# Gaussian-Splatting-Toolkit/Gaussian-Splatting-Toolkit

Measured on AMD Instinct MI355X. Metric: raster fwd+bwd Mpix/s @1080p (1M Gaussians, SH3), higher is better.
Workload: dtype f32; 1 GPU; 1000000 random Gaussians (SURVEY 8d, seed 42, scales log-U[0.0025,0.025]), SH degree 3, 1920x1080, block 16, fwd+bwd through the rasterizer autograd API; gaussians=1000000, visible=869029, list_entries=4459433, scene=uniform, cpu_bind=cpus 8-15 of NUMA node 0 (GPU 0000:0d:00.0), parallelism=single

## Files before the change

### gaussian-splatting-toolkit_amd/csrc/sort_bucket.hip

```cpp
#include "gsr_common.h"
#include "raster_common.h"
#include "tile_rows.h"

#include <algorithm>

namespace gsr_bsort {

constexpr int kChunk = 4096;
constexpr int kCap = 2048;
constexpr int kWaveCap = 1024;
constexpr int kElemBits = 12;
constexpr int kHistThreads = 1024;
constexpr int kScatterWaves = 4, kScatterThreads = 64 * kScatterWaves, kScatterItems = kChunk / kScatterThreads;
constexpr int kSortThreads = 256;

__device__ __forceinline__ unsigned depth_key(const float *__restrict__ depths, const int *__restrict__ radii,
                                              const int i) {
  const int r = radii[i];
  const unsigned bits = __float_as_uint(depths[i]);
  return r > 0 ? (bits & 0x7fffffffu) : 0u;
}

__device__ __forceinline__ void wave_minmax(unsigned &lo, unsigned &hi) {
#pragma unroll
  for (int o = 32; o > 0; o >>= 1) {
    lo = min(lo, (unsigned)__shfl_xor((int)lo, o));
    hi = max(hi, (unsigned)__shfl_xor((int)hi, o));
  }
}

__device__ __forceinline__ unsigned long long match_digit(const unsigned d, const int bits, const bool live) {
  const unsigned long long all = __ballot(live);
  unsigned lo = (unsigned)all, hi = (unsigned)(all >> 32);
#pragma unroll
  for (int bit = 0; bit < 8; ++bit) {
    if (bit < bits) {
      const unsigned one = (d >> bit) & 1u;
      const unsigned long long set = __ballot(one != 0u);
      const unsigned flip = one - 1u;
      lo &= (unsigned)set ^ flip, hi &= (unsigned)(set >> 32) ^ flip;
    }
  }
  return ((unsigned long long)hi << 32) | lo;
}

struct OctaveMap {
  unsigned base_w;
  unsigned mlo, span;
  float c;
};
constexpr unsigned kMinWidth = 16;
constexpr int kSample = 4096;

__device__ __forceinline__ unsigned bucket_of(const unsigned key, const OctaveMap *__restrict__ map) {
  if (!key) return 0u;
  const OctaveMap t = map[key >> 23];
  const unsigned mant = key & 0x7fffffu, W = t.base_w >> 16, base = t.base_w & 0xffffu;
  const unsigned d = min(mant > t.mlo ? mant - t.mlo : 0u, t.span - 1u);
  return base + min(W - 1u, (unsigned)((float)d * t.c));
}

template <int kT>
__device__ __forceinline__ void load_samples(const int n, const float *__restrict__ depths,
                                             const int *__restrict__ radii, unsigned (&sample)[kSample / kT]) {
  const int spacing = n / (kSample / 16);
#pragma unroll
  for (int q = 0; q < kSample / kT; ++q) {
    const int j = q * kT + (int)threadIdx.x;
    sample[q] = depth_key(depths, radii, (j >> 4) * spacing + (j & 15));
  }
}

template <int kT>
__device__ __forceinline__ void build_bucket_map(const unsigned (&sample)[kSample / kT], const int log2_buckets,
                                                 OctaveMap *__restrict__ map, unsigned *__restrict__ oct,
                                                 int *__restrict__ sh ) {
  const int tid = threadIdx.x, lane = tid & 63, w = tid >> 6;
  const unsigned B = 1u << log2_buckets;
  if (tid < 256) oct[tid] = 0u;
  if (tid == 0) sh[16] = -1, sh[17] = 0;
  __syncthreads();
#pragma unroll
  for (int q = 0; q < kSample / kT; ++q) {
    const unsigned long long peers = match_digit(sample[q] >> 23, 8, sample[q] != 0u);
    if (sample[q] && (peers & ((1ull << lane) - 1ull)) == 0) atomicAdd(&oct[sample[q] >> 23], (unsigned)__popcll(peers));
  }
  __syncthreads();
  {
    unsigned kmin = 0xffffffffu, kmax = 0u;
#pragma unroll
    for (int q = 0; q < kSample / kT; ++q)
      if (sample[q]) kmin = min(kmin, sample[q]), kmax = max(kmax, sample[q]);
    wave_minmax(kmin, kmax);
    if (lane == 0) atomicMin(reinterpret_cast<unsigned *>(&sh[16]), kmin), atomicMax(reinterpret_cast<unsigned *>(&sh[17]), kmax);
  }
  unsigned pop = 0;
  int first = 256, last = -1;
  if (tid < 256) {
    pop = oct[tid];
    if (pop) first = last = tid;
    unsigned sum = pop;
#pragma unroll
    for (int o = 32; o > 0; o >>= 1) {
      first = min(first, __shfl_xor(first, o));
      last = max(last, __shfl_xor(last, o));
      sum += __shfl_xor(sum, o);
    }
    if (lane == 0) sh[w] = first, sh[4 + w] = last, sh[8 + w] = (int)sum;
  }
  __syncthreads();
  first = min(min(sh[0], sh[1]), min(sh[2], sh[3]));
  last = max(max(sh[4], sh[5]), max(sh[6], sh[7]));
  const unsigned visible = (unsigned)max(sh[8] + sh[9] + sh[10] + sh[11], 1);
  int lo = max(first - 1, 0), hi = min(last + 1, 255);
  if (last < 0) lo = 1, hi = 0;
  const unsigned budget = B - 3u - kMinWidth * (unsigned)(hi - lo + 1);
  const bool inside = tid >= lo && tid <= hi;
  const unsigned width =
      (tid < 256 && inside) ? kMinWidth + (unsigned)(((unsigned long long)pop * budget) / visible) : 0u;
  unsigned incl = width;
#pragma unroll
  for (int o = 1; o < 64; o <<= 1) {
    const unsigned t = __shfl_up(incl, o);
    if (lane >= o) incl += t;
  }
  __syncthreads();
  if (tid < 256 && lane == 63) sh[w] = (int)incl;
  __syncthreads();
  if (tid < 256) {
    unsigned base = 2u + incl - width;
    for (int q = 0; q < w; ++q) base += (unsigned)sh[q];
    OctaveMap t{(1u << 16) | (tid > hi ? B - 1u : 1u), 0u, 1u, 0.f};
    if (inside) {
      const unsigned kmin = (unsigned)sh[16], kmax = (unsigned)sh[17];
      unsigned m0 = 0u, m1 = 0x7fffffu;
      if (tid == first) m0 = kmin & 0x7fffffu;
      if (tid == last) m1 = kmax & 0x7fffffu;
      const unsigned pad = (m1 - m0 + 1u) >> 5;
      if (tid == first) m0 = m0 > pad ? m0 - pad : 0u;
      if (tid == last) m1 = min(m1 + pad, 0x7fffffu);
      t.base_w = (width << 16) | base;
      t.mlo = m0, t.span = m1 - m0 + 1u;
      t.c = (float)width / (float)t.span;
    }
    map[tid] = t;
  }
  __syncthreads();
}

struct RecordArgs {
  const float *xys, *conics, *opacities;
  int tiles_x, tiles_y;
  SplatRec *recs;
};

template <bool kRecords>
__global__ __launch_bounds__(kHistThreads) void hist_kernel(const int n, const float *__restrict__ depths,
                                                            const int *__restrict__ radii, const int log2_buckets,
                                                            unsigned *__restrict__ table,
                                                            OctaveMap *__restrict__ map_out, const RecordArgs ra,
                                                            unsigned *__restrict__ zero, const int zero_words) {
  extern __shared__ unsigned h[];
  __shared__ OctaveMap map[256];
  __shared__ unsigned oct[256];
  __shared__ int sh[24];
  constexpr int kI = kChunk / kHistThreads;
  const int tid = threadIdx.x, B = 1 << log2_buckets;
  const int base = blockIdx.x * kChunk;
  for (int z = blockIdx.x * kHistThreads + tid; z < zero_words; z += gridDim.x * kHistThreads) zero[z] = 0u;
  unsigned key[kI];
  SplatIn in[kRecords ? kI : 1];
#pragma unroll
  for (int i = 0; i < kI; ++i) {
    const int idx = base + i * kHistThreads + tid;
    const unsigned k = depth_key(depths, radii, min(idx, n - 1));
    key[i] = idx < n ? k : 0xffffffffu;
    if (kRecords) in[i] = load_splat_in(min(idx, n - 1), ra.xys, radii, ra.conics, ra.opacities);
  }
  unsigned sample[kSample / kHistThreads];
  load_samples<kHistThreads>(n, depths, radii, sample);
  for (int j = tid; j < B; j += kHistThreads) h[j] = 0u;
  if (kRecords) {
#pragma unroll
    for (int i = 0; i < kI; ++i) {
      const int idx = base + i * kHistThreads + tid;
      if (idx < n) ra.recs[idx] = splat_record_from(in[i], ra.conics != nullptr, ra.tiles_x, ra.tiles_y, 16);
    }
  }
  build_bucket_map<kHistThreads>(sample, log2_buckets, map, oct, sh);
  if (blockIdx.x == 0 && tid < 256) map_out[tid] = map[tid];
#pragma unroll
  for (int i = 0; i < kI; ++i) {
    const bool culled = key[i] == 0u;
    const unsigned long long c = __ballot(culled);
    if (c && (tid & 63) == 0) atomicAdd(&h[0], (unsigned)__popcll(c));
    if (!culled && key[i] != 0xffffffffu) atomicAdd(&h[bucket_of(key[i], map)], 1u);
  }
  __syncthreads();
  unsigned *row = table + (size_t)blockIdx.x * B;
  for (int j = tid; j < B; j += kHistThreads) row[j] = h[j];
}

__global__ __launch_bounds__(256) void scan_kernel(const int chunks, const int B, unsigned *__restrict__ table,
                                                   unsigned *__restrict__ totals) {
  __shared__ unsigned part[16][16];
  const int tid = threadIdx.x, bl = tid & 15, g = tid >> 4;
  const int b = blockIdx.x * 16 + bl;
  const int per = (chunks + 15) / 16;
  const int c0 = g * per, c1 = min(chunks, c0 + per);
  if (per <= 16) {
    unsigned t[16], sum = 0;
#pragma unroll
    for (int k = 0; k < 16; ++k) {
      const unsigned v = table[(size_t)min(c0 + k, chunks - 1) * B + b];
      t[k] = c0 + k < c1 ? v : 0u;
      sum += t[k];
    }
    part[g][bl] = sum;
    __syncthreads();
    unsigned run = 0;
    for (int k = 0; k < g; ++k) run += part[k][bl];
    if (g == 15) totals[b] = run + sum;
#pragma unroll
    for (int k = 0; k < 16; ++k) {
      if (c0 + k < c1) table[(size_t)(c0 + k) * B + b] = run;
      run += t[k];
    }
    return;
  }
  unsigned sum = 0;
#pragma unroll 8
  for (int c = c0; c < c1; ++c) sum += table[(size_t)c * B + b];
  part[g][bl] = sum;
  __syncthreads();
  unsigned run = 0;
  for (int k = 0; k < g; ++k) run += part[k][bl];
  if (g == 15) totals[b] = run + sum;
#pragma unroll 8
  for (int c = c0; c < c1; ++c) {
    unsigned *q = table + (size_t)c * B + b;
    const unsigned t = *q;
    *q = run;
    run += t;
  }
}


template <int kW>
struct SortShared {
  unsigned cnt[kW][256];
  unsigned wsum[4];
};

template <int kW, int kI>
__device__ __forceinline__ unsigned rank_round(const unsigned (&v)[kI], unsigned (&rank)[kI], const int R,
                                               const int seg, const int m, const int shf, const int bits,
                                               SortShared<kW> &S) {
  const int tid = threadIdx.x, lane = tid & 63, w = tid >> 6;
  const unsigned long long lt = (1ull << lane) - 1ull;
  const unsigned mask = (1u << bits) - 1u;
#pragma unroll
  for (int k = 0; k < 4; ++k) (&S.cnt[0][0])[k * (kW * 64) + tid] = 0u;
  __syncthreads();
#pragma unroll
  for (int i = 0; i < kI; ++i) {
    if (i < R) {
      const bool live = w * seg + i * 64 + lane < m;
      unsigned d = (v[i] >> shf) & mask;
      asm volatile("" : "+v"(d)::"memory");
      const unsigned long long peers = match_digit(d, bits, live);
      const unsigned below = (unsigned)__popcll(peers & lt);
      const unsigned prev = S.cnt[w][d];
      rank[i] = prev + below;
      if (live && below == 0) S.cnt[w][d] = prev + (unsigned)__popcll(peers);
    }
  }
  __syncthreads();
  unsigned c[kW], tot = 0, incl = 0;
  if (tid < 256) {
#pragma unroll
    for (int k = 0; k < kW; ++k) c[k] = S.cnt[k][tid], tot += c[k];
    incl = tot;
#pragma unroll
    for (int o = 1; o < 64; o <<= 1) {
      const unsigned t = __shfl_up(incl, o);
      if (lane >= o) incl += t;
    }
    if (lane == 63) S.wsum[w] = incl;
  }
  __syncthreads();
  if (tid < 256) {
    unsigned run = incl - tot;
    for (int k = 0; k < w; ++k) run += S.wsum[k];
#pragma unroll
    for (int k = 0; k < kW; ++k) S.cnt[k][tid] = run, run += c[k];
  }
  __syncthreads();
  return tot;
}

template <int kW, int kI>
__device__ __forceinline__ void block_sort(unsigned (&v)[kI], const int R, const int seg, const int m, const int lo,
                                           const int nbits, unsigned *__restrict__ buf, SortShared<kW> &S) {
  const int tid = threadIdx.x, lane = tid & 63, w = tid >> 6;
  int rounds = (nbits + 7) / 8;
  for (int done = 0; done < nbits;) {
    const int bits = (nbits - done + rounds - 1) / rounds;
    const int shf = lo + done;
    unsigned rank[kI];
    rank_round<kW, kI>(v, rank, R, seg, m, shf, bits, S);
    const unsigned mask = (1u << bits) - 1u;
#pragma unroll
    for (int i = 0; i < kI; ++i)
      if (i < R && w * seg + i * 64 + lane < m) buf[S.cnt[w][(v[i] >> shf) & mask] + rank[i]] = v[i];
    __syncthreads();
#pragma unroll
    for (int i = 0; i < kI; ++i)
      if (i < R && w * seg + i * 64 + lane < m) v[i] = buf[w * seg + i * 64 + lane];
    done += bits, --rounds;
  }
}

struct Gather {
  const int *counts;
  int *cum;
  int rows, n;
};
__device__ __forceinline__ void place(int *__restrict__ order, const Gather &ga, const unsigned pos, const int id) {
  order[pos] = id;
  if (ga.counts)
    for (int r = 0; r < ga.rows; ++r) ga.cum[(size_t)r * ga.n + pos] = ga.counts[(size_t)r * ga.n + id];
}

constexpr int kSweep = 4096;

__device__ __forceinline__ unsigned long long match12(const unsigned d, const bool in) {
  const unsigned long long all = __ballot(in);
  unsigned lo = (unsigned)all, hi = (unsigned)(all >> 32);
#pragma unroll
  for (int bit = 0; bit < 12; ++bit) {
    const unsigned one = (d >> bit) & 1u;
    const unsigned long long set = __ballot(one != 0u);
    const unsigned flip = one - 1u;
    lo &= (unsigned)set ^ flip, hi &= (unsigned)(set >> 32) ^ flip;
  }
  return ((unsigned long long)hi << 32) | lo;
}

__global__ __launch_bounds__(kScatterThreads) void scatter_kernel(
    const int n, const float *__restrict__ depths, const int *__restrict__ radii,
    const OctaveMap *__restrict__ map_in, const int log2_buckets, const unsigned *__restrict__ table,
    const unsigned *__restrict__ totals,
    uint2 *__restrict__ pairs, int *__restrict__ order, unsigned *__restrict__ bucket_base,
    int *__restrict__ stats, const Gather ga) {
  __shared__ unsigned arr[kSweep];
  __shared__ unsigned short cnt[kScatterWaves][kSweep];
  __shared__ unsigned s_sum[kScatterWaves], s_max[kScatterWaves];
  __shared__ OctaveMap map[256];
  constexpr int kI = kScatterItems, seg = kChunk / kScatterWaves, kPer = kSweep / kScatterThreads;
  const int B = 1 << log2_buckets;
  const int tid = threadIdx.x, lane = tid & 63, w = tid >> 6;
  const unsigned long long lt = (1ull << lane) - 1ull;
  map[tid] = map_in[tid];
  const int base = blockIdx.x * kChunk;
  const int m = min(kChunk, n - base);
  unsigned key[kI], bkt[kI], rank[kI];
#pragma unroll
  for (int i = 0; i < kI; ++i) {
    const int e = w * seg + i * 64 + lane;
    const unsigned k = depth_key(depths, radii, base + min(e, m - 1));
    key[i] = e < m ? k : 0u;
  }
  __syncthreads();
#pragma unroll
  for (int i = 0; i < kI; ++i) bkt[i] = w * seg + i * 64 + lane < m ? bucket_of(key[i], map) : 0xffffffffu;
  unsigned first = 0, biggest = 0;
  for (int sweep = 0; sweep < B / kSweep; ++sweep) {
    unsigned tot[kPer], col[kPer];
    {
      const uint4 *tp = reinterpret_cast<const uint4 *>(totals + sweep * kSweep + tid * kPer);
      const uint4 *cp = reinterpret_cast<const uint4 *>(table + (size_t)blockIdx.x * B + sweep * kSweep + tid * kPer);
#pragma unroll
      for (int q = 0; q < kPer / 4; ++q) {
        const uint4 t = tp[q], c = cp[q];
        tot[4 * q] = t.x, tot[4 * q + 1] = t.y, tot[4 * q + 2] = t.z, tot[4 * q + 3] = t.w;
        col[4 * q] = c.x, col[4 * q + 1] = c.y, col[4 * q + 2] = c.z, col[4 * q + 3] = c.w;
      }
    }
    {
      unsigned *z = reinterpret_cast<unsigned *>(&cnt[0][0]);
#pragma unroll
      for (int q = 0; q < kScatterWaves * kSweep / 2 / kScatterThreads; ++q) z[q * kScatterThreads + tid] = 0u;
    }
    __syncthreads();
#pragma unroll
    for (int i = 0; i < kI; ++i) {
      const bool in = (bkt[i] >> 12) == (unsigned)sweep;
      unsigned d = bkt[i] & (kSweep - 1);
      asm volatile("" : "+v"(d)::"memory");
      const unsigned long long peers = match12(d, in);
      const unsigned below = (unsigned)__popcll(peers & lt);
      const unsigned prev = cnt[w][d];
      rank[i] = in ? prev + below : rank[i];
      if (in && below == 0) cnt[w][d] = (unsigned short)(prev + (unsigned)__popcll(peers));
    }
    __syncthreads();
    {
      unsigned sum = 0;
#pragma unroll
      for (int q = 0; q < kPer; ++q) {
        sum += tot[q];
        if (sweep * kSweep + tid * kPer + q > 0) biggest = max(biggest, tot[q]);
      }
      unsigned incl = sum;
#pragma unroll
      for (int o = 1; o < 64; o <<= 1) {
        const unsigned t = __shfl_up(incl, o);
        if (lane >= o) incl += t;
      }
      if (lane == 63) s_sum[w] = incl;
#pragma unroll
      for (int q = 0; q < kSweep / kScatterThreads; ++q) {
        const int d = q * kScatterThreads + tid;
        unsigned run = 0;
#pragma unroll
        for (int k = 0; k < kScatterWaves; ++k) {
          const unsigned c = cnt[k][d];
          cnt[k][d] = (unsigned short)run;
          run += c;
        }
      }
      __syncthreads();
      unsigned run = first + incl - sum;
      for (int k = 0; k < w; ++k) run += s_sum[k];
#pragma unroll
      for (int q = 0; q < kPer; ++q) {
        if (blockIdx.x == 0) bucket_base[sweep * kSweep + tid * kPer + q] = run;
        arr[tid * kPer + q] = run + col[q];
        run += tot[q];
      }
      unsigned whole = 0;
      for (int k = 0; k < kScatterWaves; ++k) whole += s_sum[k];
      first += whole;
    }
    __syncthreads();
#pragma unroll
    for (int i = 0; i < kI; ++i) {
      if ((bkt[i] >> 12) == (unsigned)sweep) {
        const unsigned d = bkt[i] & (kSweep - 1);
        const unsigned pos = arr[d] + cnt[w][d] + rank[i];
        const int id = base + w * seg + i * 64 + lane;
        if (bkt[i] == 0)
          place(order, ga, pos, id);
        else
          pairs[pos] = make_uint2(key[i], (unsigned)id);
      }
    }
    __syncthreads();
  }
  if (blockIdx.x == 0) {
#pragma unroll
    for (int o = 32; o > 0; o >>= 1) biggest = max(biggest, (unsigned)__shfl_xor((int)biggest, o));
    if (lane == 0) s_max[w] = biggest;
    __syncthreads();
    if (tid == 0) {
      unsigned mx = 0;
      for (int k = 0; k < kScatterWaves; ++k) mx = max(mx, s_max[k]);
      stats[0] = (int)mx;
      bucket_base[B] = first;
    }
  }
}

struct WaveShared {
  unsigned buf[kWaveCap], ids[kWaveCap], cnt[256];
};
struct BlockShared {
  unsigned buf[kCap], idL[kCap];
  SortShared<4> S;
};

template <int kI>
__device__ __forceinline__ bool wave_sort(const unsigned s, const int m, const uint2 *__restrict__ pairs,
                                          int *__restrict__ order, const Gather &ga, WaveShared &W) {
  constexpr int kEBits = kI == 1 ? 6 : kI == 2 ? 7 : kI == 4 ? 8 : kI == 8 ? 9 : 10;
  const int lane = threadIdx.x & 63;
  const unsigned long long lt = (1ull << lane) - 1ull;
  unsigned v[kI], rank[kI];
  unsigned kmin = 0xffffffffu, kmax = 0u;
#pragma unroll
  for (int i = 0; i < kI; ++i) {
    const int e = i * 64 + lane;
    const uint2 pr = pairs[s + min(e, m - 1)];
    if (e < m) W.ids[e] = pr.y;
    v[i] = pr.x;
    kmin = min(kmin, pr.x), kmax = max(kmax, pr.x);
  }
  wave_minmax(kmin, kmax);
  kmin = __builtin_amdgcn_readfirstlane(kmin), kmax = __builtin_amdgcn_readfirstlane(kmax);
  const int lowbits = kmax > kmin ? 32 - __clz((int)(kmax - kmin)) : 0;
  if (lowbits + kEBits > 32) return false;
#pragma unroll
  for (int i = 0; i < kI; ++i) {
    const int e = i * 64 + lane;
    v[i] = e < m ? ((v[i] - kmin) << kEBits) | (unsigned)e : 0u;
  }
  int rounds = (lowbits + 7) / 8;
  for (int done = 0; done < lowbits;) {
    const int bits = (lowbits - done + rounds - 1) / rounds;
    const int shf = kEBits + done;
    const unsigned mask = (1u << bits) - 1u;
#pragma unroll
    for (int q = 0; q < 4; ++q) W.cnt[q * 64 + lane] = 0u;
#pragma unroll
    for (int i = 0; i < kI; ++i) {
      {
        const bool live = i * 64 + lane < m;
        unsigned d = (v[i] >> shf) & mask;
        asm volatile("" : "+v"(d)::"memory");
        const unsigned long long peers = match_digit(d, bits, live);
        const unsigned below = (unsigned)__popcll(peers & lt);
        const unsigned prev = W.cnt[d];
        rank[i] = prev + below;
        if (live && below == 0) W.cnt[d] = prev + (unsigned)__popcll(peers);
      }
    }
    {
      const unsigned c0 = W.cnt[4 * lane], c1 = W.cnt[4 * lane + 1], c2 = W.cnt[4 * lane + 2],
                     c3 = W.cnt[4 * lane + 3];
      const unsigned tot = c0 + c1 + c2 + c3;
      unsigned incl = tot;
#pragma unroll
      for (int o = 1; o < 64; o <<= 1) {
        const unsigned t = __shfl_up(incl, o);
        if (lane >= o) incl += t;
      }
      const unsigned ex = incl - tot;
      W.cnt[4 * lane] = ex, W.cnt[4 * lane + 1] = ex + c0, W.cnt[4 * lane + 2] = ex + c0 + c1,
                   W.cnt[4 * lane + 3] = ex + c0 + c1 + c2;
    }
#pragma unroll
    for (int i = 0; i < kI; ++i)
      if (i * 64 + lane < m) W.buf[W.cnt[(v[i] >> shf) & mask] + rank[i]] = v[i];
#pragma unroll
    for (int i = 0; i < kI; ++i)
      if (i * 64 + lane < m) v[i] = W.buf[i * 64 + lane];
    done += bits, --rounds;
  }
#pragma unroll
  for (int i = 0; i < kI; ++i)
    if (i * 64 + lane < m) place(order, ga, s + i * 64 + lane, (int)W.ids[v[i] & ((1u << kEBits) - 1u)]);
  return true;
}

__device__ __noinline__ void sort_large_bucket(const unsigned s, const unsigned m, uint2 *pairs, uint2 *pairs2,
                                               int *__restrict__ order, const Gather &ga, unsigned *run,
                                               SortShared<4> &S) {
  constexpr int kI = 4, kTile = kI * kSortThreads;
  const int tid = threadIdx.x, lane = tid & 63, w = tid >> 6;
  unsigned sub;
  int lowbits;
  {
    unsigned lo = 0xffffffffu, hi = 0u;
    for (unsigned e = tid; e < m; e += kSortThreads) {
      const unsigned k = pairs[s + e].x;
      lo = min(lo, k), hi = max(hi, k);
    }
    wave_minmax(lo, hi);
    if (lane == 0) S.cnt[0][w] = lo, S.cnt[1][w] = hi;
    __syncthreads();
    lo = min(min(S.cnt[0][0], S.cnt[0][1]), min(S.cnt[0][2], S.cnt[0][3]));
    hi = max(max(S.cnt[1][0], S.cnt[1][1]), max(S.cnt[1][2], S.cnt[1][3]));
    __syncthreads();
    if (lo == hi) {
      for (unsigned e = tid; e < m; e += kSortThreads) place(order, ga, s + e, (int)pairs[s + e].y);
      return;
    }
    sub = lo, lowbits = 32 - __clz((int)(hi - lo));
  }
  uint2 *src = pairs, *dst = pairs2;
  int rounds = (lowbits + 7) / 8;
  for (int done = 0; done < lowbits;) {
    const int bits = (lowbits - done + rounds - 1) / rounds;
    const unsigned mask = (1u << bits) - 1u;
    run[tid] = 0u;
    __syncthreads();
    for (unsigned e = tid; e < m; e += kSortThreads)
      atomicAdd(&run[((src[s + e].x - sub) >> done) & mask], 1u);
    __syncthreads();
    {
      const unsigned c = run[tid];
      unsigned incl = c;
#pragma unroll
      for (int o = 1; o < 64; o <<= 1) {
        const unsigned t = __shfl_up(incl, o);
        if (lane >= o) incl += t;
      }
      if (lane == 63) S.wsum[w] = incl;
      __syncthreads();
      unsigned ex = incl - c;
      for (int k = 0; k < w; ++k) ex += S.wsum[k];
      run[tid] = ex;
      __syncthreads();
    }
    for (unsigned t0 = 0; t0 < m; t0 += kTile) {
      const int mt = (int)min((unsigned)kTile, m - t0);
      constexpr int R = kI, seg = R * 64;
      unsigned v[kI], rank[kI];
      uint2 pr[kI];
#pragma unroll
      for (int i = 0; i < kI; ++i) {
        const int e = w * seg + i * 64 + lane;
        pr[i] = src[s + t0 + min(e, mt - 1)];
        v[i] = e < mt ? (pr[i].x - sub) >> done : 0u;
      }
      const unsigned tot = rank_round<4, kI>(v, rank, R, seg, mt, 0, bits, S);
#pragma unroll
      for (int i = 0; i < kI; ++i) {
        const int e = w * seg + i * 64 + lane;
        if (i < R && e < mt) {
          const unsigned d = v[i] & mask;
          dst[s + run[d] + S.cnt[w][d] - S.cnt[0][d] + rank[i]] = pr[i];
        }
      }
      __syncthreads();
      run[tid] += tot;
      __syncthreads();
    }
    uint2 *t = src;
    src = dst, dst = t;
    done += bits, --rounds;
    __threadfence_block();
  }
  for (unsigned e = tid; e < m; e += kSortThreads) place(order, ga, s + e, (int)src[s + e].y);
}

template <int kI>
__device__ __forceinline__ bool block_bucket(const unsigned s, const int m, const uint2 *__restrict__ pairs,
                                             int *__restrict__ order, const Gather &ga, BlockShared &L) {
  const int tid = threadIdx.x, lane = tid & 63, w = tid >> 6;
  constexpr int seg = kI * 64;
  unsigned v[kI];
  unsigned kmin = 0xffffffffu, kmax = 0u;
#pragma unroll
  for (int i = 0; i < kI; ++i) {
    const int e = w * seg + i * 64 + lane;
    const uint2 pr = pairs[s + min(e, m - 1)];
    if (e < m) L.idL[e] = pr.y;
    v[i] = pr.x;
    kmin = min(kmin, pr.x), kmax = max(kmax, pr.x);
  }
  wave_minmax(kmin, kmax);
  if (lane == 0) L.S.cnt[0][w] = kmin, L.S.cnt[1][w] = kmax;
  __syncthreads();
  kmin = min(min(L.S.cnt[0][0], L.S.cnt[0][1]), min(L.S.cnt[0][2], L.S.cnt[0][3]));
  kmax = max(max(L.S.cnt[1][0], L.S.cnt[1][1]), max(L.S.cnt[1][2], L.S.cnt[1][3]));
  kmin = __builtin_amdgcn_readfirstlane(kmin), kmax = __builtin_amdgcn_readfirstlane(kmax);
  __syncthreads();
  const int lowbits = kmax > kmin ? 32 - __clz((int)(kmax - kmin)) : 0;
  if (lowbits + kElemBits > 32) return false;
#pragma unroll
  for (int i = 0; i < kI; ++i) {
    const int e = w * seg + i * 64 + lane;
    v[i] = e < m ? ((v[i] - kmin) << kElemBits) | (unsigned)e : 0u;
  }
  block_sort<4, kI>(v, kI, seg, m, kElemBits, lowbits, L.buf, L.S);
#pragma unroll
  for (int i = 0; i < kI; ++i) {
    const int e = w * seg + i * 64 + lane;
    if (e < m) place(order, ga, s + e, (int)L.idL[v[i] & ((1u << kElemBits) - 1u)]);
  }
  return true;
}

__global__ __launch_bounds__(kSortThreads) void bucket_sort_kernel(const int B,
                                                                   const unsigned *__restrict__ bucket_base,
                                                                   uint2 *pairs, uint2 *pairs2,
                                                                   int *__restrict__ order, const Gather ga) {
  __shared__ union {
    WaveShared wave[4];
    BlockShared blk;
  } L;
  __shared__ unsigned s_start[5];
  __shared__ int s_left[4];
  const int tid = threadIdx.x, w = tid >> 6;
  const int b0 = 1 + 4 * blockIdx.x;
  if (tid < 5) s_start[tid] = bucket_base[min(b0 + tid, B)];
  __syncthreads();
  {
    const unsigned sw = __builtin_amdgcn_readfirstlane(s_start[w]);
    const unsigned mw = __builtin_amdgcn_readfirstlane(s_start[w + 1]) - sw;
    const int b = b0 + __builtin_amdgcn_readfirstlane(w);
    bool left = mw > 0 && b < B;
    if (left && mw <= (unsigned)kWaveCap && b != 1 && b != B - 1) {
      if (mw <= 64)
        left = !wave_sort<1>(sw, (int)mw, pairs, order, ga, L.wave[w]);
      else if (mw <= 128)
        left = !wave_sort<2>(sw, (int)mw, pairs, order, ga, L.wave[w]);
      else if (mw <= 256)
        left = !wave_sort<4>(sw, (int)mw, pairs, order, ga, L.wave[w]);
      else if (mw <= 512)
        left = !wave_sort<8>(sw, (int)mw, pairs, order, ga, L.wave[w]);
      else
        left = !wave_sort<16>(sw, (int)mw, pairs, order, ga, L.wave[w]);
    }
    if ((tid & 63) == 0) s_left[w] = left;
  }
  __syncthreads();
  if (!(s_left[0] | s_left[1] | s_left[2] | s_left[3])) return;
// ... 79 lines not shown
```

### gaussian-splatting-toolkit_amd/csrc/tile_partition2.hip

```cpp
#include "gsr_common.h"
#include "raster_common.h"
#include "tile_rows.h"

int gsr_tile_bases(int num_tiles, unsigned *totals, int *tile_bins, hipStream_t s);

namespace gsr_p2 {

constexpr int kSlab = 256;
constexpr int kGroup = 64;
constexpr int kItems = 1024;
constexpr int kMaskBlocks = 256;
constexpr int kChunk = 4096;
constexpr int kMaxDim = 1024;

struct Dims {
  int n, slabs, groups, tiles_x, tiles_y, txp;
};

struct SlabItems {
  int pref[kSlab];
  int gid[kSlab];
  SplatRec rec[kSlab];
  RowParams par[kSlab];
};

__device__ __forceinline__ int block_excl(const int v, int *__restrict__ wsum, int &total) {
  const int lane = threadIdx.x & 63, w = threadIdx.x >> 6;
  int incl = v;
#pragma unroll
  for (int o = 1; o < 64; o <<= 1) {
    const int t = __shfl_up(incl, o);
    if (lane >= o) incl += t;
  }
  __syncthreads();
  if (lane == 63) wsum[w] = incl;
  __syncthreads();
  int base = 0;
  for (int k = 0; k < w; ++k) base += wsum[k];
  total = wsum[0] + wsum[1] + wsum[2] + wsum[3];
  return base + incl - v;
}

__device__ __forceinline__ long long block_excl64(const long long v, long long *__restrict__ wsum, long long &total) {
  const int lane = threadIdx.x & 63, w = threadIdx.x >> 6;
  long long incl = v;
#pragma unroll
  for (int o = 1; o < 64; o <<= 1) {
    const long long t = __shfl_up(incl, o);
    if (lane >= o) incl += t;
  }
  __syncthreads();
  if (lane == 63) wsum[w] = incl;
  __syncthreads();
  long long base = 0;
  for (int k = 0; k < w; ++k) base += wsum[k];
  total = wsum[0] + wsum[1] + wsum[2] + wsum[3];
  return base + incl - v;
}

__device__ __forceinline__ int load_slab(SlabItems &W, int *__restrict__ wsum, const int i, const int n,
                                         const int *__restrict__ order, const SplatRec *__restrict__ recs) {
  const int tid = threadIdx.x;
  SplatRec rec{0.f, 0.f, 1.f, 0.f, 1.f, -1.f, 0u, 0u};
  int g = 0;
  if (i < n) {
    g = order[i];
    rec = recs[g];
  }
  const int h = (int)(rec.box1 >> 16);
  int total;
  W.pref[tid] = block_excl(h, wsum, total) + h;
  W.gid[tid] = g;
  W.rec[tid] = rec;
  W.par[tid] = make_row_params(rec);
  __syncthreads();
  return total;
}

__device__ __forceinline__ void item_of(const SlabItems &W, const int q, const int total, int &k, int &ty, int &t0,
                                        int &t1) {
  k = 0;
#pragma unroll
  for (int step = kSlab / 2; step > 0; step >>= 1)
    if (W.pref[k + step - 1] <= q) k += step;
  k = k < kSlab - 1 ? k : kSlab - 1;
  const SplatRec r = W.rec[k];
  ty = (int)(r.box0 >> 16) + q - (k ? W.pref[k - 1] : 0);
  t0 = t1 = 0;
  if (q < total) row_range(r, W.par[k], ty, t0, t1);
}

__global__ __launch_bounds__(kSlab) void rowcount_kernel(const Dims D, const int *__restrict__ order,
                                                         const SplatRec *__restrict__ recs, int *__restrict__ tableC) {
  __shared__ SlabItems W;
  __shared__ int wsum[4];
  extern __shared__ int rowcnt[];
  const int tid = threadIdx.x, slab = blockIdx.x;
  for (int r = tid; r < D.tiles_y; r += kSlab) rowcnt[r] = 0;
  const int total = load_slab(W, wsum, slab * kSlab + tid, D.n, order, recs);
  for (int q = tid; q < total; q += kSlab) {
    int k, ty, t0, t1;
    item_of(W, q, total, k, ty, t0, t1);
    if (t1 > t0) atomicAdd(&rowcnt[ty], t1 - t0);
  }
  __syncthreads();
  for (int r = tid; r < D.tiles_y; r += kSlab) tableC[(size_t)r * D.slabs + slab] = rowcnt[r];
}

__global__ __launch_bounds__(1024) void rowscan_kernel(const Dims D, const int *__restrict__ tableC,
                                                       int *__restrict__ tableA, int *__restrict__ rowtot) {
  __shared__ int wsum[16];
  const int tid = threadIdx.x, lane = tid & 63, w = tid >> 6, row = blockIdx.x;
  const int *src = tableC + (size_t)row * D.slabs;
  int *dst = tableA + (size_t)row * D.slabs;
  int carry = 0;
  for (int base = 0; base < D.slabs; base += 1024) {
    const int i = base + tid;
    const int v = i < D.slabs ? src[i] : 0;
    int incl = v;
#pragma unroll
    for (int o = 1; o < 64; o <<= 1) {
      const int t = __shfl_up(incl, o);
      if (lane >= o) incl += t;
    }
    if (lane == 63) wsum[w] = incl;
    __syncthreads();
    int before = carry, all = 0;
    for (int k = 0; k < 16; ++k) {
      if (k < w) before += wsum[k];
      all += wsum[k];
    }
    if (i < D.slabs) dst[i] = before + incl - v;
    carry += all;
    __syncthreads();
  }
  if (tid == 0) rowtot[row] = carry;
}

template <class F>
__device__ __forceinline__ int scan_rows(const int ny, F f, int *out, const bool with_total, int *wsum) {
  const int tid = threadIdx.x, lane = tid & 63, w = tid >> 6;
  int carry = 0;
  for (int base = 0; base < ny; base += kSlab) {
    const int r = base + tid;
    const int v = r < ny ? f(r) : 0;
    int incl = v;
#pragma unroll
    for (int o = 1; o < 64; o <<= 1) {
      const int t = __shfl_up(incl, o);
      if (lane >= o) incl += t;
    }
    __syncthreads();
    if (lane == 63) wsum[w] = incl;
    __syncthreads();
    int before = carry;
    for (int k = 0; k < w; ++k) before += wsum[k];
    if (r < ny) out[r] = before + incl - v;
    carry += wsum[0] + wsum[1] + wsum[2] + wsum[3];
  }
  __syncthreads();
  if (with_total && tid == 0) out[ny] = carry;
  return carry;
}

__global__ __launch_bounds__(kSlab) void emit_kernel(const Dims D, const int capacity, const int *__restrict__ order,
                                                     const SplatRec *__restrict__ recs, const int *__restrict__ tableA,
                                                     const int *__restrict__ rowtot, int *__restrict__ row_start,
                                                     int *__restrict__ row_chunk_start, int *__restrict__ count_out,
                                                     unsigned short *__restrict__ tx_out, int *__restrict__ gid_out) {
  constexpr int kR = kItems / kSlab;
  __shared__ SlabItems W;
  __shared__ unsigned it_a[kItems];
  __shared__ unsigned it_b[kItems];
  __shared__ unsigned short sorted[kItems];
  __shared__ int sout[kItems + 1];
  __shared__ unsigned long long smask[kMaskBlocks];
  __shared__ int blkfirst[kMaskBlocks];
  __shared__ int wsum[4];
  __shared__ long long wsum64[4];
  extern __shared__ int rows_lds[];
  const int ny = D.tiles_y;
  int *wcnt = rows_lds;
  int *bent = wcnt + 4 * ny;
  int *bentc = bent + ny;
  int *gcur = bentc + ny;
  const int tid = threadIdx.x, lane = tid & 63, w = tid >> 6, slab = blockIdx.x;
  const unsigned long long lt = (1ull << lane) - 1ull;
  const bool few_rows = ny <= kSlab;
  int my_total = 0, my_prefix = 0;
  if (few_rows && tid < ny) my_total = rowtot[tid], my_prefix = tableA[(size_t)tid * D.slabs + slab];
  const int total = load_slab(W, wsum, slab * kSlab + tid, D.n, order, recs);
  const int entries = scan_rows(ny, [&](int r) { return few_rows ? my_total : rowtot[r]; }, gcur, false, wsum);
  if (slab == 0) {
    for (int r = tid; r < ny; r += kSlab) row_start[r] = gcur[r];
    if (tid == 0) {
      row_start[ny] = entries;
      if (count_out) *count_out = entries;
    }
    scan_rows(ny, [&](int r) {
      const int s0 = min(gcur[r], capacity), s1 = min(gcur[r] + rowtot[r], capacity);
      return (s1 - s0 + kChunk - 1) / kChunk;
    }, row_chunk_start, true, wsum);
  }
  for (int r = tid; r < ny; r += kSlab) gcur[r] += few_rows ? my_prefix : tableA[(size_t)r * D.slabs + slab];
  int row_bits = 1;
  while ((1 << row_bits) < ny) ++row_bits;
  const int rp = (ny + kSlab - 1) / kSlab;

  for (int qa = 0; qa < total; qa += kItems) {
    const int nb = total - qa < kItems ? total - qa : kItems;
    for (int r = tid; r < 4 * ny; r += kSlab) wcnt[r] = 0;
    for (int r = tid; r < ny; r += kSlab) bentc[r] = 0;
    __syncthreads();
    const int per = ((nb + 255) >> 8) << 6;
    int rank[kR], myrow[kR];
#pragma unroll
    for (int r = 0; r < kR; ++r) {
      myrow[r] = -1;
      rank[r] = 0;
      if (r * 64 >= per) continue;
      const int idx = w * per + r * 64 + lane;
      int k = 0, ty = 0, t0 = 0, t1 = 0;
      if (idx < nb) item_of(W, qa + idx, total, k, ty, t0, t1);
      const int cnt = t1 - t0;
      if (idx < nb) {
        it_a[idx] = (unsigned)ty | ((unsigned)t0 << 16);
        it_b[idx] = (unsigned)cnt | ((unsigned)k << 16);
      }
      const bool live = idx < nb && cnt > 0;
      unsigned long long peers = __ballot(live);
      for (int bit = 0; bit < row_bits; ++bit) {
        const bool b = (ty >> bit) & 1;
        const unsigned long long set = __ballot(b);
        peers &= b ? set : ~set;
      }
      const int below = __popcll(peers & lt);
      const int prev = live ? wcnt[w * ny + ty] : 0;
      rank[r] = prev + below;
      if (live && below == 0) wcnt[w * ny + ty] = prev + __popcll(peers);
      if (live) atomicAdd(&bentc[ty], cnt);
      myrow[r] = live ? ty : -1;
    }
    __syncthreads();
    int nplaced, E;
    {
      int ci = 0, ce = 0;
      for (int j = 0; j < rp; ++j) {
        const int r = tid * rp + j;
        if (r < ny) {
          ci += wcnt[r] + wcnt[ny + r] + wcnt[2 * ny + r] + wcnt[3 * ny + r];
          ce += bentc[r];
        }
      }
      long long tot;
      const long long ex = block_excl64(((long long)ce << 32) | (long long)ci, wsum64, tot);
      int run_i = (int)(ex & 0xffffffffll), run_e = (int)(ex >> 32);
      nplaced = (int)(tot & 0xffffffffll);
      E = (int)(tot >> 32);
      for (int j = 0; j < rp; ++j) {
        const int r = tid * rp + j;
        if (r < ny) {
#pragma unroll
          for (int q = 0; q < 4; ++q) {
            const int c = wcnt[q * ny + r];
            wcnt[q * ny + r] = run_i;
            run_i += c;
          }
          bent[r] = run_e;
          run_e += bentc[r];
        }
      }
    }
    __syncthreads();
#pragma unroll
    for (int r = 0; r < kR; ++r)
      if (myrow[r] >= 0) sorted[wcnt[w * ny + myrow[r]] + rank[r]] = (unsigned short)(w * per + r * 64 + lane);
    __syncthreads();
    {
      int c[kR], sum = 0;
#pragma unroll
      for (int j = 0; j < kR; ++j) {
        const int sidx = tid * kR + j;
        c[j] = sidx < nplaced ? (int)(it_b[sorted[sidx]] & 0xffffu) : 0;
        sum += c[j];
      }
      int tot;
      int run = block_excl(sum, wsum, tot);
#pragma unroll
      for (int j = 0; j < kR; ++j) {
        const int sidx = tid * kR + j;
        if (sidx < nplaced) sout[sidx] = run;
        run += c[j];
      }
      if (tid == 0) sout[nplaced] = E;
    }
    const int nblk = (E + 63) >> 6;
    const bool use_masks = nblk <= kMaskBlocks;
    if (use_masks) {
      if (tid < nblk) smask[tid] = 0ull;
      __syncthreads();
      for (int sidx = tid; sidx < nplaced; sidx += kSlab) atomicOr(&smask[sout[sidx] >> 6], 1ull << (sout[sidx] & 63));
      __syncthreads();
      const int c = tid < nblk ? __popcll(smask[tid]) : 0;
      int tot;
      const int ex = block_excl(c, wsum, tot);
      if (tid < nblk) blkfirst[tid] = ex;
      __syncthreads();
      for (int j0 = 0; j0 < E; j0 += 4 * kSlab) {
        int jj[4], lo[4];
#pragma unroll
        for (int u = 0; u < 4; ++u) {
          jj[u] = j0 + u * kSlab + tid;
          const int jc = jj[u] < E ? jj[u] : E - 1;
          lo[u] = blkfirst[jc >> 6] + __popcll(smask[jc >> 6] & ((2ull << (jc & 63)) - 1ull)) - 1;
        }
        unsigned a[4], b[4];
        int so[4];
#pragma unroll
        for (int u = 0; u < 4; ++u) {
          const int si = sorted[lo[u]];
          a[u] = it_a[si];
          b[u] = it_b[si];
          so[u] = sout[lo[u]];
        }
        long long pos[4];
        int gidv[4];
#pragma unroll
        for (int u = 0; u < 4; ++u) {
          const int row = (int)(a[u] & 0xffffu);
          pos[u] = (long long)gcur[row] + (jj[u] - bent[row]);
          gidv[u] = W.gid[b[u] >> 16];
        }
#pragma unroll
        for (int u = 0; u < 4; ++u)
          if (jj[u] < E && pos[u] < capacity) {
            tx_out[pos[u]] = (unsigned short)((int)(a[u] >> 16) + (jj[u] - so[u]));
            gid_out[pos[u]] = gidv[u];
          }
      }
    } else {
      __syncthreads();
      for (int j = tid; j < E; j += kSlab) {
        int lo = 0, hi = nplaced;
        while (hi - lo > 1) {
          const int mid = (lo + hi) >> 1;
          if (sout[mid] <= j) lo = mid;
          else hi = mid;
        }
        const unsigned a = it_a[sorted[lo]], b = it_b[sorted[lo]];
        const int row = (int)(a & 0xffffu), t0 = (int)(a >> 16), k = (int)(b >> 16);
        const long long pos = (long long)gcur[row] + (j - bent[row]);
        if (pos < capacity) {
          tx_out[pos] = (unsigned short)(t0 + (j - sout[lo]));
          gid_out[pos] = W.gid[k];
        }
      }
    }
    __syncthreads();
    for (int r = tid; r < ny; r += kSlab) gcur[r] += bentc[r];
    __syncthreads();
  }
}

__device__ __forceinline__ bool chunk_slice(const Dims &D, const int capacity, const int c,
                                            const int *__restrict__ row_start,
                                            const int *__restrict__ row_chunk_start, int &row, int &beg, int &end) {
  if (c >= row_chunk_start[D.tiles_y]) return false;
  int lo = 0, hi = D.tiles_y;
  while (hi - lo > 1) {
    const int mid = (lo + hi) >> 1;
    if (row_chunk_start[mid] <= c) lo = mid;
    else hi = mid;
  }
  row = lo;
  const int rs = min(row_start[row], capacity), re = min(row_start[row + 1], capacity);
  beg = rs + (c - row_chunk_start[row]) * kChunk;
  end = min(beg + kChunk, re);
  return beg < end;
}

__global__ __launch_bounds__(256) void colhist_kernel(const Dims D, const int capacity,
                                                      const int *__restrict__ row_start,
                                                      const int *__restrict__ row_chunk_start,
                                                      const unsigned short *__restrict__ tx_in,
                                                      int *__restrict__ tableB) {
  __shared__ int h[kMaxDim];
  int row, beg, end;
  if (!chunk_slice(D, capacity, blockIdx.x, row_start, row_chunk_start, row, beg, end)) return;
  for (int t = threadIdx.x; t < D.txp; t += 256) h[t] = 0;
  __syncthreads();
  const uint2 *in4 = reinterpret_cast<const uint2 *>(tx_in);
  for (int g = (beg >> 2) + threadIdx.x; g * 4 < end; g += 256) {
    const uint2 v = in4[g];
    const int e = g * 4;
    if (e >= beg && e < end) atomicAdd(&h[v.x & 0xffffu], 1);
    if (e + 1 >= beg && e + 1 < end) atomicAdd(&h[v.x >> 16], 1);
    if (e + 2 >= beg && e + 2 < end) atomicAdd(&h[v.y & 0xffffu], 1);
    if (e + 3 >= beg && e + 3 < end) atomicAdd(&h[v.y >> 16], 1);
  }
  __syncthreads();
  int *out = tableB + (size_t)blockIdx.x * D.txp;
  for (int t = threadIdx.x; t < D.txp; t += 256) out[t] = h[t];
}

__global__ __launch_bounds__(256) void colscan_kernel(const Dims D, const int *__restrict__ row_chunk_start,
                                                      int *__restrict__ tableB, unsigned *__restrict__ tile_cnt) {
  __shared__ int part[4][64];
  const int lane = threadIdx.x & 63, q = threadIdx.x >> 6;
  const int tx = blockIdx.x * 64 + lane, row = blockIdx.y;
  const int c0 = row_chunk_start[row], c1 = row_chunk_start[row + 1];
  const int per = (c1 - c0 + 3) >> 2;
  const int cb = min(c0 + q * per, c1), ce = min(cb + per, c1);
  const bool live = tx < D.tiles_x;
  int sum = 0;
  if (live)
    for (int c = cb; c < ce; ++c) sum += tableB[(size_t)c * D.txp + tx];
  part[q][lane] = sum;
  __syncthreads();
  int run = 0;
  for (int k = 0; k < q; ++k) run += part[k][lane];
  if (!live) return;
  for (int c = cb; c < ce; ++c) {
    int *p = tableB + (size_t)c * D.txp + tx;
    const int v = *p;
    *p = run;
    run += v;
  }
  if (q == 3) tile_cnt[(size_t)row * D.tiles_x + tx] = (unsigned)run;
}

__global__ __launch_bounds__(1024) void colscan_row_kernel(const Dims D, const int capacity,
                                                           const int *__restrict__ row_start,
                                                           const int *__restrict__ row_chunk_start,
                                                           int *__restrict__ tableB, unsigned *__restrict__ tile_base,
                                                           int *__restrict__ tile_bins) {
  __shared__ int part[4][256];
  __shared__ int s_tot[256];
  __shared__ int wsum[4];
  const int tid = threadIdx.x, lane = tid & 63, wv = tid >> 6, cg = wv & 3, q = wv >> 2;
  const int tx = cg * 64 + lane, row = blockIdx.x;
  const int c0 = row_chunk_start[row], c1 = row_chunk_start[row + 1];
  const int per = (c1 - c0 + 3) >> 2;
  const int cb = min(c0 + q * per, c1), ce = min(cb + per, c1);
  const bool live = tx < D.tiles_x;
  int sum = 0;
  if (live)
    for (int c = cb; c < ce; ++c) sum += tableB[(size_t)c * D.txp + tx];
  part[q][tx] = sum;
  __syncthreads();
  int run = 0;
  for (int k = 0; k < q; ++k) run += part[k][tx];
  if (live)
    for (int c = cb; c < ce; ++c) {
      int *p = tableB + (size_t)c * D.txp + tx;
      const int v = *p;
      *p = run;
      run += v;
    }
  if (q == 3) s_tot[tx] = live ? run : 0;
  __syncthreads();
  if (tid < 256) {
    const int v = s_tot[tid];
    int incl = v;
#pragma unroll
    for (int o = 1; o < 64; o <<= 1) {
      const int t = __shfl_up(incl, o);
      if (lane >= o) incl += t;
    }
    if (lane == 63) wsum[wv] = incl;
    s_tot[tid] = incl - v;
  }
  __syncthreads();
  if (tid < D.tiles_x) {
    int before = 0;
    for (int k = 0; k < (tid >> 6); ++k) before += wsum[k];
    const int v = part[0][tid] + part[1][tid] + part[2][tid] + part[3][tid];
    const int base = min(row_start[row], capacity) + before + s_tot[tid];
    const size_t tile = (size_t)row * D.tiles_x + tid;
    tile_base[tile] = (unsigned)base;
    tile_bins[2 * tile] = v ? base : 0;
    tile_bins[2 * tile + 1] = v ? base + v : 0;
  }
}

template <int CMAX>
__global__ __launch_bounds__(256) void colscatter_kernel(const Dims D, const int capacity,
                                                         const int *__restrict__ row_start,
                                                         const int *__restrict__ row_chunk_start,
                                                         const unsigned short *__restrict__ tx_in,
                                                         const int *__restrict__ gid_in,
                                                         const int *__restrict__ tableB,
                                                         const unsigned *__restrict__ tile_base,
                                                         int *__restrict__ ids_out) {
  constexpr int kRounds = kChunk / 256;
  __shared__ unsigned short s_stx[kChunk];
  __shared__ int s_gid[kChunk];
  __shared__ int loff[CMAX];
  __shared__ int wcnt[4][CMAX];
  __shared__ int wsum[4];
  int row, beg, end;
  if (!chunk_slice(D, capacity, blockIdx.x, row_start, row_chunk_start, row, beg, end)) return;
  const int tid = threadIdx.x, lane = tid & 63, w = tid >> 6, cnt = end - beg;
  const unsigned long long lt = (1ull << lane) - 1ull;
  for (int t = tid; t < 4 * CMAX; t += 256) (&wcnt[0][0])[t] = 0;
  __syncthreads();
  int key_bits = 1;
  while ((1 << key_bits) < D.tiles_x) ++key_bits;
  int key[kRounds], gid[kRounds], rank[kRounds];
#pragma unroll
  for (int r = 0; r < kRounds; ++r) {
    const int e = w * (kChunk / 4) + r * 64 + lane;
    const bool live = e < cnt;
    key[r] = live ? (int)tx_in[beg + e] : -1;
    gid[r] = live ? gid_in[beg + e] : 0;
  }
#pragma unroll
  for (int r = 0; r < kRounds; ++r) {
    const bool live = key[r] >= 0;
    const unsigned k = live ? (unsigned)key[r] : 0u;
    unsigned long long peers = __ballot(live);
    for (int bit = 0; bit < key_bits; ++bit) {
      const bool b = (k >> bit) & 1u;
      const unsigned long long set = __ballot(b);
      peers &= b ? set : ~set;
    }
    const int below = __popcll(peers & lt);
    const int prev = live ? wcnt[w][k] : 0;
    rank[r] = prev + below;
    if (live && below == 0) wcnt[w][k] = prev + __popcll(peers);
  }
  __syncthreads();
  {
    constexpr int kPer = CMAX / 256;
    int v[kPer], s = 0;
#pragma unroll
    for (int j = 0; j < kPer; ++j) {
      const int c = tid * kPer + j;
      v[j] = wcnt[0][c] + wcnt[1][c] + wcnt[2][c] + wcnt[3][c];
      s += v[j];
    }
    int incl = s;
#pragma unroll
    for (int o = 1; o < 64; o <<= 1) {
      const int t = __shfl_up(incl, o);
      if (lane >= o) incl += t;
    }
    if (lane == 63) wsum[w] = incl;
    __syncthreads();
    int base = incl - s;
    for (int k = 0; k < w; ++k) base += wsum[k];
#pragma unroll
    for (int j = 0; j < kPer; ++j) {
      const int c = tid * kPer + j;
      loff[c] = base;
      int run = base;
#pragma unroll
      for (int q = 0; q < 4; ++q) {
        const int n = wcnt[q][c];
        wcnt[q][c] = run;
        run += n;
      }
      base += v[j];
    }
  }
  __syncthreads();
#pragma unroll
  for (int r = 0; r < kRounds; ++r) {
    if (key[r] >= 0) {
      const int pos = wcnt[w][key[r]] + rank[r];
      s_gid[pos] = gid[r];
      s_stx[pos] = (unsigned short)key[r];
    }
  }
  __syncthreads();
  const int *pre = tableB + (size_t)blockIdx.x * D.txp;
  const unsigned *tb = tile_base + (size_t)row * D.tiles_x;
  for (int t = tid; t < D.tiles_x; t += 256) loff[t] = (int)(tb[t] + (unsigned)pre[t] - (unsigned)loff[t]);
  __syncthreads();
  for (int j = tid; j < cnt; j += 256) ids_out[(unsigned)loff[s_stx[j]] + (unsigned)j] = s_gid[j];
}

inline size_t align_up(size_t v) { return (v + 255) & ~(size_t)255; }

struct Layout {
  size_t tableC, tableA, gtot, row_start, row_chunk_start, tx, gid, tableB, tile_cnt, total;
  int chunk_slots;
};
inline Layout make_layout(const Dims &D, int capacity) {
  Layout L{};
  size_t off = 0;
  auto take = [&](size_t bytes) {
    const size_t o = off;
    off += align_up(bytes);
    return o;
  };
  L.tableC = take(4 * (size_t)D.slabs * D.tiles_y);
  L.tableA = take(4 * (size_t)D.slabs * D.tiles_y);
  L.gtot = take(4 * (size_t)D.tiles_y * (D.groups > 1 ? D.groups : 1));
  L.row_start = take(4 * (size_t)(D.tiles_y + 1));
  L.row_chunk_start = take(4 * (size_t)(D.tiles_y + 1));
  L.tx = take(2 * (size_t)capacity + 8);
  L.gid = take(4 * (size_t)capacity);
  L.chunk_slots = capacity / kChunk + D.tiles_y + 1;
  L.tableB = take(4 * (size_t)L.chunk_slots * D.txp);
  L.tile_cnt = take(4 * (size_t)D.tiles_x * D.tiles_y);
  L.total = off;
  return L;
}
inline Dims make_dims(int n, int tiles_x, int tiles_y) {
  Dims D;
  D.n = n;
  D.slabs = (n + kSlab - 1) / kSlab;
  D.groups = (D.slabs + kGroup - 1) / kGroup;
  D.tiles_x = tiles_x;
  D.tiles_y = tiles_y;
  D.txp = (tiles_x + 3) & ~3;
  return D;
}

}

bool gsr_tile_partition2_supported(int tiles_x, int tiles_y) {
  return tiles_x >= 1 && tiles_y >= 1 && tiles_x <= gsr_p2::kMaxDim && tiles_y < gsr_p2::kMaxDim;
}

size_t gsr_tile_partition2_workspace_bytes(int n, int capacity, int tiles_x, int tiles_y) {
  using namespace gsr_p2;
  if (n <= 0 || capacity <= 0) return 0;
  return make_layout(make_dims(n, tiles_x, tiles_y), capacity).total;
}

int gsr_tile_partition2(int n, int capacity, const int *order, const void *recs, int tiles_x, int tiles_y,
                        int *ids_sorted, int *tile_bins, int *count_out, void *workspace, size_t workspace_bytes,
                        hipStream_t s) {
  using namespace gsr_p2;
  if (!gsr_tile_partition2_supported(tiles_x, tiles_y)) {
    gsr_set_error("tile_partition2: a %d x %d tile grid is not supported", tiles_x, tiles_y);
    return GSR_EINVAL;
  }
  const Dims D = make_dims(n, tiles_x, tiles_y);
  const Layout L = make_layout(D, capacity);
  if (workspace_bytes < L.total) {
    gsr_set_error("tile_partition2: workspace %zu < %zu bytes", workspace_bytes, L.total);
    return GSR_ENOMEM;
  }
  char *ws = static_cast<char *>(workspace);
  int *tableC = reinterpret_cast<int *>(ws + L.tableC), *tableA = reinterpret_cast<int *>(ws + L.tableA);
  int *gtot = reinterpret_cast<int *>(ws + L.gtot), *row_start = reinterpret_cast<int *>(ws + L.row_start);
  int *row_chunk_start = reinterpret_cast<int *>(ws + L.row_chunk_start);
  unsigned short *txs = reinterpret_cast<unsigned short *>(ws + L.tx);
  int *gids = reinterpret_cast<int *>(ws + L.gid), *tableB = reinterpret_cast<int *>(ws + L.tableB);
  unsigned *tile_cnt = reinterpret_cast<unsigned *>(ws + L.tile_cnt);
  const SplatRec *R = static_cast<const SplatRec *>(recs);
  hipLaunchKernelGGL(rowcount_kernel, dim3(D.slabs), dim3(kSlab), 4 * (size_t)tiles_y, s, D, order, R, tableC);
  hipLaunchKernelGGL(rowscan_kernel, dim3(tiles_y), dim3(1024), 0, s, D, (const int *)tableC, tableA, gtot);
  hipLaunchKernelGGL(emit_kernel, dim3(D.slabs), dim3(kSlab), 28 * (size_t)tiles_y, s, D, capacity, order, R,
                     (const int *)tableA, (const int *)gtot, row_start, row_chunk_start, count_out, txs, gids);
  hipLaunchKernelGGL(colhist_kernel, dim3(L.chunk_slots), dim3(256), 0, s, D, capacity, (const int *)row_start,
                     (const int *)row_chunk_start, (const unsigned short *)txs, tableB);
  if (tiles_x <= 256) {
    hipLaunchKernelGGL(colscan_row_kernel, dim3(tiles_y), dim3(1024), 0, s, D, capacity, (const int *)row_start,
                       (const int *)row_chunk_start, tableB, tile_cnt, tile_bins);
  } else {
    hipLaunchKernelGGL(colscan_kernel, dim3(gsr_cdiv(tiles_x, 64), tiles_y), dim3(256), 0, s, D,
                       (const int *)row_chunk_start, tableB, tile_cnt);
    int rc = gsr_tile_bases(tiles_x * tiles_y, tile_cnt, tile_bins, s);
    if (rc != GSR_OK) return rc;
  }
  if (tiles_x <= 256)
    hipLaunchKernelGGL(colscatter_kernel<256>, dim3(L.chunk_slots), dim3(256), 0, s, D, capacity,
                       (const int *)row_start, (const int *)row_chunk_start, (const unsigned short *)txs,
                       (const int *)gids, (const int *)tableB, (const unsigned *)tile_cnt, ids_sorted);
  else
    hipLaunchKernelGGL(colscatter_kernel<1024>, dim3(L.chunk_slots), dim3(256), 0, s, D, capacity,
                       (const int *)row_start, (const int *)row_chunk_start, (const unsigned short *)txs,
                       (const int *)gids, (const int *)tableB, (const unsigned *)tile_cnt, ids_sorted);
  GSR_CHECK_LAUNCH("tile_partition2");
  return GSR_OK;
}
```

Baseline: 2075 Mpix/s.

## Cut LDS and register pressure in bucket scatter and tile partition kernels

Doubles the scatter kernel to 8 waves per block. The octave map now borrows the arr shared buffer, and the per-wave count prefix is done on packed 32-bit pairs. In the tile emit kernel, slab records and item buffers share one union, and the slab records are reloaded when a row has more than one item pass. Tile ranks are packed into the upper half of the key register, and asm barriers pin the rank values so the compiler does not rematerialize them. The aim is lower LDS and VGPR use for better occupancy, at the risk of extra record reloads and correctness subtleties from the aliased buffers.

```diff
diff --git a/gaussian-splatting-toolkit_amd/csrc/sort_bucket.hip b/gaussian-splatting-toolkit_amd/csrc/sort_bucket.hip
--- a/gaussian-splatting-toolkit_amd/csrc/sort_bucket.hip
+++ b/gaussian-splatting-toolkit_amd/csrc/sort_bucket.hip
@@ -11,7 +11,7 @@
 constexpr int kWaveCap = 1024;
 constexpr int kElemBits = 12;
 constexpr int kHistThreads = 1024;
-constexpr int kScatterWaves = 4, kScatterThreads = 64 * kScatterWaves, kScatterItems = kChunk / kScatterThreads;
+constexpr int kScatterWaves = 8, kScatterThreads = 64 * kScatterWaves, kScatterItems = kChunk / kScatterThreads;
 constexpr int kSortThreads = 256;
 
 __device__ __forceinline__ unsigned depth_key(const float *__restrict__ depths, const int *__restrict__ radii,
@@ -272,6 +272,7 @@
       const unsigned below = (unsigned)__popcll(peers & lt);
       const unsigned prev = S.cnt[w][d];
       rank[i] = prev + below;
+      asm volatile("" : "+v"(rank[i]));
       if (live && below == 0) S.cnt[w][d] = prev + (unsigned)__popcll(peers);
     }
   }
@@ -356,12 +357,13 @@
   __shared__ unsigned arr[kSweep];
   __shared__ unsigned short cnt[kScatterWaves][kSweep];
   __shared__ unsigned s_sum[kScatterWaves], s_max[kScatterWaves];
-  __shared__ OctaveMap map[256];
+  static_assert(sizeof(OctaveMap) * 256 <= sizeof(arr), "the map borrows arr");
+  OctaveMap *map = reinterpret_cast<OctaveMap *>(arr);
   constexpr int kI = kScatterItems, seg = kChunk / kScatterWaves, kPer = kSweep / kScatterThreads;
   const int B = 1 << log2_buckets;
   const int tid = threadIdx.x, lane = tid & 63, w = tid >> 6;
   const unsigned long long lt = (1ull << lane) - 1ull;
-  map[tid] = map_in[tid];
+  if (tid < 256) map[tid] = map_in[tid];
   const int base = blockIdx.x * kChunk;
   const int m = min(kChunk, n - base);
   unsigned key[kI], bkt[kI], rank[kI];
@@ -402,6 +404,7 @@
       const unsigned below = (unsigned)__popcll(peers & lt);
       const unsigned prev = cnt[w][d];
       rank[i] = in ? prev + below : rank[i];
+      asm volatile("" : "+v"(rank[i]));
       if (in && below == 0) cnt[w][d] = (unsigned short)(prev + (unsigned)__popcll(peers));
     }
     __syncthreads();
@@ -419,14 +422,15 @@
         if (lane >= o) incl += t;
       }
       if (lane == 63) s_sum[w] = incl;
-#pragma unroll
-      for (int q = 0; q < kSweep / kScatterThreads; ++q) {
-        const int d = q * kScatterThreads + tid;
+      unsigned *c2 = reinterpret_cast<unsigned *>(&cnt[0][0]);
+#pragma unroll
+      for (int q = 0; q < kSweep / 2 / kScatterThreads; ++q) {
+        const int d2 = q * kScatterThreads + tid;
         unsigned run = 0;
 #pragma unroll
         for (int k = 0; k < kScatterWaves; ++k) {
-          const unsigned c = cnt[k][d];
-          cnt[k][d] = (unsigned short)run;
+          const unsigned c = c2[k * (kSweep / 2) + d2];
+          c2[k * (kSweep / 2) + d2] = run;
           run += c;
         }
       }
@@ -522,6 +526,7 @@
         const unsigned below = (unsigned)__popcll(peers & lt);
         const unsigned prev = W.cnt[d];
         rank[i] = prev + below;
+        asm volatile("" : "+v"(rank[i]));
         if (live && below == 0) W.cnt[d] = prev + (unsigned)__popcll(peers);
       }
     }
@@ -554,7 +559,7 @@
 }
 
 __device__ __noinline__ void sort_large_bucket(const unsigned s, const unsigned m, uint2 *pairs, uint2 *pairs2,
-                                               int *__restrict__ order, const Gather &ga, unsigned *run,
+                                               int *__restrict__ order, const Gather ga, unsigned *run,
                                                SortShared<4> &S) {
   constexpr int kI = 4, kTile = kI * kSortThreads;
   const int tid = threadIdx.x, lane = tid & 63, w = tid >> 6;
diff --git a/gaussian-splatting-toolkit_amd/csrc/tile_partition2.hip b/gaussian-splatting-toolkit_amd/csrc/tile_partition2.hip
--- a/gaussian-splatting-toolkit_amd/csrc/tile_partition2.hip
+++ b/gaussian-splatting-toolkit_amd/csrc/tile_partition2.hip
@@ -24,6 +24,23 @@
   RowParams par[kSlab];
 };
 
+struct EmitSlab {
+  int pref[kSlab];
+  int gid[kSlab];
+  union {
+    struct {
+      SplatRec rec[kSlab];
+      RowParams par[kSlab];
+    };
+    struct {
+      unsigned it_a[kItems];
+      unsigned it_b[kItems];
+      unsigned short sorted[kItems];
+      int blkfirst[kMaskBlocks];
+    };
+  };
+};
+
 __device__ __forceinline__ int block_excl(const int v, int *__restrict__ wsum, int &total) {
   const int lane = threadIdx.x & 63, w = threadIdx.x >> 6;
   int incl = v;
@@ -58,7 +75,8 @@
   return base + incl - v;
 }
 
-__device__ __forceinline__ int load_slab(SlabItems &W, int *__restrict__ wsum, const int i, const int n,
+template <class Slab>
+__device__ __forceinline__ int load_slab(Slab &W, int *__restrict__ wsum, const int i, const int n,
                                          const int *__restrict__ order, const SplatRec *__restrict__ recs) {
   const int tid = threadIdx.x;
   SplatRec rec{0.f, 0.f, 1.f, 0.f, 1.f, -1.f, 0u, 0u};
@@ -77,7 +95,8 @@
   return total;
 }
 
-__device__ __forceinline__ void item_of(const SlabItems &W, const int q, const int total, int &k, int &ty, int &t0,
+template <class Slab>
+__device__ __forceinline__ void item_of(const Slab &W, const int q, const int total, int &k, int &ty, int &t0,
                                         int &t1) {
   k = 0;
 #pragma unroll
@@ -169,13 +188,12 @@
                                                      int *__restrict__ row_chunk_start, int *__restrict__ count_out,
                                                      unsigned short *__restrict__ tx_out, int *__restrict__ gid_out) {
   constexpr int kR = kItems / kSlab;
-  __shared__ SlabItems W;
-  __shared__ unsigned it_a[kItems];
-  __shared__ unsigned it_b[kItems];
-  __shared__ unsigned short sorted[kItems];
+  __shared__ EmitSlab W;
+  unsigned *it_a = W.it_a, *it_b = W.it_b;
+  unsigned short *sorted = W.sorted;
+  int *blkfirst = W.blkfirst;
   __shared__ int sout[kItems + 1];
   __shared__ unsigned long long smask[kMaskBlocks];
-  __shared__ int blkfirst[kMaskBlocks];
   __shared__ int wsum[4];
   __shared__ long long wsum64[4];
   extern __shared__ int rows_lds[];
@@ -209,10 +227,29 @@
 
   for (int qa = 0; qa < total; qa += kItems) {
     const int nb = total - qa < kItems ? total - qa : kItems;
+    if (qa > 0) {
+      const int i = slab * kSlab + tid;
+      SplatRec rec{0.f, 0.f, 1.f, 0.f, 1.f, -1.f, 0u, 0u};
+      if (i < D.n) rec = recs[W.gid[tid]];
+      W.rec[tid] = rec;
+      W.par[tid] = make_row_params(rec);
+    }
     for (int r = tid; r < 4 * ny; r += kSlab) wcnt[r] = 0;
     for (int r = tid; r < ny; r += kSlab) bentc[r] = 0;
     __syncthreads();
     const int per = ((nb + 255) >> 8) << 6;
+    unsigned ia[kR], ib[kR];
+#pragma unroll
+    for (int r = 0; r < kR; ++r) {
+      ia[r] = ib[r] = 0u;
+      if (r * 64 >= per) continue;
+      const int idx = w * per + r * 64 + lane;
+      int k = 0, ty = 0, t0 = 0, t1 = 0;
+      if (idx < nb) item_of(W, qa + idx, total, k, ty, t0, t1);
+      ia[r] = (unsigned)ty | ((unsigned)t0 << 16);
+      ib[r] = (unsigned)(t1 - t0) | ((unsigned)k << 16);
+    }
+    __syncthreads();
     int rank[kR], myrow[kR];
 #pragma unroll
     for (int r = 0; r < kR; ++r) {
@@ -220,12 +257,10 @@
       rank[r] = 0;
       if (r * 64 >= per) continue;
       const int idx = w * per + r * 64 + lane;
-      int k = 0, ty = 0, t0 = 0, t1 = 0;
-      if (idx < nb) item_of(W, qa + idx, total, k, ty, t0, t1);
-      const int cnt = t1 - t0;
+      const int ty = (int)(ia[r] & 0xffffu), cnt = (int)(ib[r] & 0xffffu);
       if (idx < nb) {
-        it_a[idx] = (unsigned)ty | ((unsigned)t0 << 16);
-        it_b[idx] = (unsigned)cnt | ((unsigned)k << 16);
+        it_a[idx] = ia[r];
+        it_b[idx] = ib[r];
       }
       const bool live = idx < nb && cnt > 0;
       unsigned long long peers = __ballot(live);
@@ -237,6 +272,7 @@
       const int below = __popcll(peers & lt);
       const int prev = live ? wcnt[w * ny + ty] : 0;
       rank[r] = prev + below;
+      asm volatile("" : "+v"(rank[r]));
       if (live && below == 0) wcnt[w * ny + ty] = prev + __popcll(peers);
       if (live) atomicAdd(&bentc[ty], cnt);
       myrow[r] = live ? ty : -1;
@@ -506,18 +542,20 @@
   __syncthreads();
   int key_bits = 1;
   while ((1 << key_bits) < D.tiles_x) ++key_bits;
-  int key[kRounds], gid[kRounds], rank[kRounds];
+  constexpr unsigned kDead = 0xffffu;
+  unsigned key[kRounds];
+  int gid[kRounds];
 #pragma unroll
   for (int r = 0; r < kRounds; ++r) {
     const int e = w * (kChunk / 4) + r * 64 + lane;
     const bool live = e < cnt;
-    key[r] = live ? (int)tx_in[beg + e] : -1;
+    key[r] = live ? (unsigned)tx_in[beg + e] : kDead;
     gid[r] = live ? gid_in[beg + e] : 0;
   }
 #pragma unroll
   for (int r = 0; r < kRounds; ++r) {
-    const bool live = key[r] >= 0;
-    const unsigned k = live ? (unsigned)key[r] : 0u;
+    const bool live = key[r] != kDead;
+    const unsigned k = live ? key[r] : 0u;
     unsigned long long peers = __ballot(live);
     for (int bit = 0; bit < key_bits; ++bit) {
       const bool b = (k >> bit) & 1u;
@@ -526,7 +564,8 @@
     }
     const int below = __popcll(peers & lt);
     const int prev = live ? wcnt[w][k] : 0;
-    rank[r] = prev + below;
+    key[r] |= (unsigned)(prev + below) << 16;
+    asm volatile("" : "+v"(key[r]));
     if (live && below == 0) wcnt[w][k] = prev + __popcll(peers);
   }
   __syncthreads();
@@ -566,10 +605,11 @@
   __syncthreads();
 #pragma unroll
   for (int r = 0; r < kRounds; ++r) {
-    if (key[r] >= 0) {
-      const int pos = wcnt[w][key[r]] + rank[r];
+    const unsigned c = key[r] & 0xffffu;
+    if (c != kDead) {
+      const int pos = wcnt[w][c] + (int)(key[r] >> 16);
       s_gid[pos] = gid[r];
-      s_stx[pos] = (unsigned short)key[r];
+      s_stx[pos] = (unsigned short)c;
     }
   }
   __syncthreads();
```

After: 2107 Mpix/s (median of 6 runs). +1.5%, better.
